# muhtutorials/wireguard

Hardware: AMD Instinct MI355X
Metric: device-resident payload GiB/s, Internet checksum, 64k×1500B batch (higher is better)
Workload: dtype u8; 1 GPU; 65536 x 1500-B tcp4 frames per GPU, validate (checksumValid, gro.go:554-612) per step, BASELINE.json configs[1]; packets_per_gpu=65536, frame_len=1500, global_batch_bytes=98304000, mode=validate, rotated_copies=4, frame_stride=1500, streams=2, parallelism=shard1 (no collective)

## Files before the change

wireguard_amd/csrc/api.cpp:

```cpp
#include <hip/hip_runtime.h>

#include <algorithm>

#include <cstdarg>
#include <cstdio>
#include <cstdlib>
#include <cstring>
#include <mutex>
#include <string>

#include "../../include/wgcsum.h"
#include "wgcs_ctx.h"
#include "wgcs_kernels.h"

using namespace wgcs;

namespace wgcs {

namespace {
thread_local const wgcs_ctx* tls_err_ctx = nullptr;
thread_local char tls_err[512];
}

int set_err(wgcs_ctx* ctx, int code, const char* fmt, ...) {
  if (ctx) {
    va_list ap;
    va_start(ap, fmt);
    vsnprintf(tls_err, sizeof tls_err, fmt, ap);
    va_end(ap);
    tls_err_ctx = ctx;
  }
  return code;
}

int hip_fail(wgcs_ctx* ctx, hipError_t e, const char* what) {
  return set_err(ctx, WGCS_ERR_HIP, "%s: %s", what, hipGetErrorString(e));
}

int ensure_dev(wgcs_ctx* ctx, DevBuf& b, size_t bytes) {
  if (bytes <= b.cap) return WGCS_OK;
  if (b.ptr) hipFree(b.ptr);
  b.ptr = nullptr;
  b.cap = 0;
  size_t want = bytes < 4096 ? 4096 : bytes + bytes / 4;
  hipError_t e = hipMalloc(&b.ptr, want);
  if (e != hipSuccess) return hip_fail(ctx, e, "hipMalloc");
  b.cap = want;
  return WGCS_OK;
}

int ensure_pinned(wgcs_ctx* ctx, HostBuf& b, size_t bytes) {
  if (bytes <= b.cap) return WGCS_OK;
  if (b.ptr) hipHostFree(b.ptr);
  b.ptr = nullptr;
  b.cap = 0;
  size_t want = bytes < 4096 ? 4096 : bytes + bytes / 4;
  hipError_t e = hipHostMalloc(&b.ptr, want, hipHostMallocDefault);
  if (e != hipSuccess) return hip_fail(ctx, e, "hipHostMalloc");
  void* d = nullptr;
  e = hipHostGetDevicePointer(&d, b.ptr, 0);
  if (e != hipSuccess || d != b.ptr) {
    hipHostFree(b.ptr);
    b.ptr = nullptr;
    return e != hipSuccess ? hip_fail(ctx, e, "hipHostGetDevicePointer")
                           : set_err(ctx, WGCS_ERR_HIP, "pinned memory is not mapped at its host address");
  }
  b.cap = want;
  return WGCS_OK;
}

bool host_mapped_locked(wgcs_ctx* ctx, const void* p, size_t n) {
  const uintptr_t a = (uintptr_t)p, b = a + n;
  for (const auto& r : ctx->host_allocs)
    if (a >= r.first && b <= r.second && b >= a) return true;
  return false;
}

bool host_mapped(wgcs_ctx* ctx, const void* p, size_t n) {
  std::lock_guard<std::mutex> g(ctx->host_mu);
  return host_mapped_locked(ctx, p, n);
}

}

extern "C" {

int wgcs_abi_version(void) { return WGCS_ABI_VERSION; }

int wgcs_device_count(int* count) {
  if (!count) return WGCS_ERR_INVALID_ARG;
  int n = 0;
  hipError_t e = hipGetDeviceCount(&n);
  if (e != hipSuccess) {
    *count = 0;
    return WGCS_ERR_NO_DEVICE;
  }
  *count = n;
  return WGCS_OK;
}

int wgcs_init(int device, wgcs_ctx** out) {
  if (!out) return WGCS_ERR_INVALID_ARG;
  *out = nullptr;
  int n = 0;
  if (hipGetDeviceCount(&n) != hipSuccess || n <= 0) return WGCS_ERR_NO_DEVICE;
  if (device < 0 || device >= n) return WGCS_ERR_INVALID_ARG;
  wgcs_ctx* ctx = new (std::nothrow) wgcs_ctx();
  if (!ctx) return WGCS_ERR_NOMEM;
  ctx->device = device;
  hipError_t e = hipSetDevice(device);
  if (e == hipSuccess) e = hipStreamCreateWithFlags(&ctx->stream, hipStreamDefault);
  hipDeviceProp_t prop;
  if (e == hipSuccess) e = hipGetDeviceProperties(&prop, device);
  for (int j = 1; j < WGCS_MAX_BATCH_STREAMS && e == hipSuccess; ++j)
    e = hipEventCreateWithFlags(&ctx->join_ev[j], hipEventDisableTiming);
  if (e != hipSuccess) {
    for (hipEvent_t ev : ctx->join_ev)
      if (ev) hipEventDestroy(ev);
    if (ctx->stream) hipStreamDestroy(ctx->stream);
    delete ctx;
    return WGCS_ERR_HIP;
  }
  ctx->num_cu = prop.multiProcessorCount;
  const char* bpc = getenv("WGCS_BLOCKS_PER_CU");
  if (bpc && atoi(bpc) > 0) ctx->tune.blocks_per_cu = atoi(bpc);
  const char* unr = getenv("WGCS_UNROLL");
  if (unr && atoi(unr) > 0) ctx->tune.unroll = atoi(unr);
  const char* lpp = getenv("WGCS_LANES_PER_PKT");
  if (lpp && (atoi(lpp) == 64 || atoi(lpp) == 32 || atoi(lpp) == 16)) ctx->tune.lanes_per_pkt = atoi(lpp);
  const char* nt = getenv("WGCS_NT");
  if (nt) ctx->tune.nt = atoi(nt) ? 1 : 0;
  const char* xc = getenv("WGCS_XCD");
  if (xc) ctx->tune.xcd = atoi(xc) ? 1 : 0;
  const char* al = getenv("WGCS_ALIGN");
  if (al && (atoi(al) == 16 || atoi(al) == 32 || atoi(al) == 64 || atoi(al) == 128)) ctx->tune.align = atoi(al);
  *out = ctx;
  return WGCS_OK;
}

int wgcs_host_alloc(wgcs_ctx* ctx, size_t bytes, void** p) {
  if (!ctx || !p || bytes == 0) return WGCS_ERR_INVALID_ARG;
  *p = nullptr;
  hipSetDevice(ctx->device);
  const size_t n = (bytes + 15) & ~(size_t)15;
  void* h = nullptr;
  hipError_t e = hipHostMalloc(&h, n, hipHostMallocCoherent);
  if (e != hipSuccess) return hip_fail(ctx, e, "wgcs_host_alloc");
  void* d = nullptr;
  e = hipHostGetDevicePointer(&d, h, 0);
  if (e != hipSuccess || d != h) {
    hipHostFree(h);
    return e != hipSuccess ? hip_fail(ctx, e, "hipHostGetDevicePointer")
                           : set_err(ctx, WGCS_ERR_HIP, "pinned memory is not mapped at its host address");
  }
  std::lock_guard<std::mutex> g(ctx->host_mu);
  ctx->host_allocs.emplace_back((uintptr_t)h, (uintptr_t)h + n);
  *p = h;
  return WGCS_OK;
}

int wgcs_host_free(wgcs_ctx* ctx, void* p) {
  if (!ctx || !p) return WGCS_ERR_INVALID_ARG;
  {
    std::lock_guard<std::mutex> g(ctx->host_mu);
    auto& v = ctx->host_allocs;
    auto it = std::find_if(v.begin(), v.end(), [&](const std::pair<uintptr_t, uintptr_t>& r) {
      return r.first == (uintptr_t)p;
    });
    if (it == v.end()) return set_err(ctx, WGCS_ERR_INVALID_ARG, "wgcs_host_free: not a wgcs_host_alloc pointer");
    for (wgcs_wstager* ws : ctx->wstagers)
      if (wstager_references(ws, it->first, it->second))
        return set_err(ctx, WGCS_ERR_NOT_READY, "wgcs_host_free: a write-stager slot still reads this memory");
    v.erase(it);
  }
  const hipError_t e = hipHostFree(p);
  return e == hipSuccess ? WGCS_OK : hip_fail(ctx, e, "hipHostFree");
}

int wgcs_destroy(wgcs_ctx* ctx) {
  if (!ctx) return WGCS_ERR_INVALID_ARG;
  {
    std::lock_guard<std::mutex> g(ctx->host_mu);
    if (!ctx->wstagers.empty() || !ctx->stagers.empty())
      return set_err(ctx, WGCS_ERR_INVALID_ARG,
                     "wgcs_destroy: %zu read stager(s) and %zu write stager(s) still alive: destroy them first",
                     ctx->stagers.size(), ctx->wstagers.size());
  }
  hipSetDevice(ctx->device);
  if (ctx->stream) hipStreamSynchronize(ctx->stream);
  for (const auto& r : ctx->host_allocs) hipHostFree((void*)r.first);
  for (DevBuf* b : {&ctx->d_arena, &ctx->d_pkts, &ctx->d_init, &ctx->d_out, &ctx->d_out2, &ctx->d_aux})
    if (b->ptr) hipFree(b->ptr);
  for (HostBuf* b : {&ctx->h_stage, &ctx->h_meta, &ctx->h_out})
    if (b->ptr) hipHostFree(b->ptr);
  if (ctx->stream) hipStreamDestroy(ctx->stream);
  for (hipEvent_t ev : ctx->join_ev)
    if (ev) hipEventDestroy(ev);
  delete ctx;
  return WGCS_OK;
}

const char* wgcs_strerror(int status) {
  switch (status) {
    case WGCS_OK: return "ok";
    case WGCS_ERR_INVALID_ARG: return "invalid argument";
    case WGCS_ERR_SHORT_BUFFER: return "short buffer";
    case WGCS_ERR_TOO_MANY_SEGMENTS: return "too many segments";
    case WGCS_ERR_INVALID_OFFSET: return "invalid offset";
    case WGCS_ERR_UNSUPPORTED_GSO: return "unsupported virtio GSO type";
    case WGCS_ERR_IP_GSO_MISMATCH: return "IP header version / GSO type mismatch";
    case WGCS_ERR_BAD_IP_VERSION: return "invalid IP header version";
    case WGCS_ERR_PACKET_TOO_SHORT: return "packet is too short";
    case WGCS_ERR_TCP_HDR_LEN: return "TCP header length is invalid";
    case WGCS_ERR_HDR_LEN: return "length of packet < virtioNetHdr.hdrLen";
    case WGCS_ERR_CSUM_OFFSET: return "end of checksum offset exceeds packet length";
    case WGCS_ERR_READ_OVERFLOW: return "read length overflows bufs element length";
    case WGCS_ERR_OUT_OF_RANGE: return "slice bounds out of range";
    case WGCS_ERR_BATCH_FULL: return "staging batch full";
    case WGCS_ERR_NOT_READY: return "batch not submitted or already recycled";
    case WGCS_ERR_CMSG: return "error parsing socket control message";
    case WGCS_ERR_SPLIT_OVERFLOW: return "splitting coalesced packet resulted in overflow";
    case WGCS_ERR_AUTH: return "chacha20poly1305: message authentication failed";
    case WGCS_ERR_SOURCE: return "packet with disallowed source address";
    case WGCS_ERR_REPLAY: return "replayed or out-of-window counter";
    case WGCS_ERR_MAC1: return "received packet with invalid mac1";
    case WGCS_ERR_LOW_ORDER: return "bad input point: low order point";
    case WGCS_ERR_NO_PEER: return "no running peer with this public key";
    case WGCS_ERR_HIP: return "HIP runtime error";
    case WGCS_ERR_NOMEM: return "out of memory";
    case WGCS_ERR_NO_DEVICE: return "no HIP device";
    default: return "unknown status";
  }
}

const char* wgcs_last_error(wgcs_ctx* ctx) { return ctx && tls_err_ctx == ctx ? tls_err : ""; }

int wgcs_num_cu(wgcs_ctx* ctx) { return ctx ? ctx->num_cu : WGCS_ERR_INVALID_ARG; }

int wgcs_sync(wgcs_ctx* ctx) {
  if (!ctx) return WGCS_ERR_INVALID_ARG;
  std::lock_guard<std::mutex> g(ctx->mu);
  hipSetDevice(ctx->device);
  hipError_t e = hipStreamSynchronize(ctx->stream);
  return e == hipSuccess ? WGCS_OK : hip_fail(ctx, e, "hipStreamSynchronize");
}

int wgcs_checksum_batch(wgcs_ctx* ctx, int mode, unsigned flags, uint8_t* d_arena, const wgcs_pkt* d_pkts,
                        const uint64_t* d_initial, uint32_t n, void* d_out, void* stream) {
  if (!ctx) return WGCS_ERR_INVALID_ARG;
  if (mode < WGCS_MODE_FOLD || mode > WGCS_MODE_IP4HDR) return set_err(ctx, WGCS_ERR_INVALID_ARG, "bad mode %d", mode);
  if (n == 0) return WGCS_OK;
  if (!d_arena || !d_pkts || !d_out) return set_err(ctx, WGCS_ERR_INVALID_ARG, "NULL pointer");
  std::lock_guard<std::mutex> g(ctx->mu);
  hipSetDevice(ctx->device);
  hipStream_t s = stream ? (hipStream_t)stream : ctx->stream;
  hipError_t e = launch_checksum_batch(mode, flags, d_arena, d_pkts, d_initial, n, d_out, s, ctx->num_cu, ctx->tune);
  return e == hipSuccess ? WGCS_OK : hip_fail(ctx, e, "checksum_batch launch");
}

int wgcs_checksum_batches(wgcs_ctx* ctx, int mode, unsigned flags, const wgcs_batch* batches, uint32_t n_batches,
                          void* const* streams, uint32_t n_streams, void* ev_begin, void* ev_end) {
  if (!ctx) return WGCS_ERR_INVALID_ARG;
  if (mode < WGCS_MODE_FOLD || mode > WGCS_MODE_IP4HDR) return set_err(ctx, WGCS_ERR_INVALID_ARG, "bad mode %d", mode);
  if (n_streams > WGCS_MAX_BATCH_STREAMS || (n_streams && !streams) || (n_batches && !batches))
    return set_err(ctx, WGCS_ERR_INVALID_ARG, "bad stream list (%u streams)", n_streams);
  for (uint32_t k = 0; k < n_batches; ++k)
    if (batches[k].n && (!batches[k].arena || !batches[k].pkts || !batches[k].out))
      return set_err(ctx, WGCS_ERR_INVALID_ARG, "batch %u: NULL pointer", k);
  std::lock_guard<std::mutex> g(ctx->mu);
  hipSetDevice(ctx->device);
  const uint32_t ns = n_streams ? n_streams : 1;
  hipStream_t st[WGCS_MAX_BATCH_STREAMS];
  for (uint32_t j = 0; j < ns; ++j) st[j] = n_streams && streams[j] ? (hipStream_t)streams[j] : ctx->stream;
  hipError_t e = hipSuccess;
  if (ev_begin && (e = hipEventRecord((hipEvent_t)ev_begin, st[0])) != hipSuccess) return hip_fail(ctx, e, "ev_begin");
  for (uint32_t k = 0; k < n_batches; ++k) {
    const uint32_t j = k % ns;
    if (ev_begin && j != 0 && k < ns && st[j] != st[0] &&
        (e = hipStreamWaitEvent(st[j], (hipEvent_t)ev_begin, 0)) != hipSuccess)
      return hip_fail(ctx, e, "stream wait");
    const wgcs_batch& b = batches[k];
    e = launch_checksum_batch(mode, flags, b.arena, b.pkts, b.initial, b.n, b.out, st[j], ctx->num_cu, ctx->tune);
    if (e != hipSuccess) return hip_fail(ctx, e, "checksum_batches launch");
  }
  if (ev_end) {
    const uint32_t used = n_batches < ns ? n_batches : ns;
    for (uint32_t j = 1; j < used; ++j) {
      if (st[j] == st[0]) continue;
      if ((e = hipEventRecord(ctx->join_ev[j], st[j])) != hipSuccess ||
          (e = hipStreamWaitEvent(st[0], ctx->join_ev[j], 0)) != hipSuccess)
        return hip_fail(ctx, e, "stream join");
    }
    if ((e = hipEventRecord((hipEvent_t)ev_end, st[0])) != hipSuccess) return hip_fail(ctx, e, "ev_end");
  }
  return WGCS_OK;
}

int wgcs_stream_wait_flag(wgcs_ctx* ctx, void* stream, const uint32_t* flag, uint32_t value) {
  if (!ctx || !flag || ((uintptr_t)flag & 3u)) return WGCS_ERR_INVALID_ARG;
  if (!host_mapped(ctx, flag, sizeof(uint32_t)))
    return set_err(ctx, WGCS_ERR_INVALID_ARG, "wgcs_stream_wait_flag: flag is not wgcs_host_alloc memory");
  std::lock_guard<std::mutex> g(ctx->mu);
  hipSetDevice(ctx->device);
  hipStream_t s = stream ? (hipStream_t)stream : ctx->stream;
  const hipError_t e = hipStreamWaitValue32(s, const_cast<uint32_t*>(flag), value, hipStreamWaitValueEq, 0xFFFFFFFFu);
  return e == hipSuccess ? WGCS_OK : hip_fail(ctx, e, "hipStreamWaitValue32");
}

constexpr size_t kZeroCopyMax = 1u << 20;

int wgcs_checksum_batch_host(wgcs_ctx* ctx, int mode, unsigned flags, uint8_t* h_arena, size_t arena_len,
                             const wgcs_pkt* h_pkts, const uint64_t* h_initial, uint32_t n, void* h_out) {
  if (!ctx) return WGCS_ERR_INVALID_ARG;
  if (mode < WGCS_MODE_FOLD || mode > WGCS_MODE_IP4HDR) return set_err(ctx, WGCS_ERR_INVALID_ARG, "bad mode %d", mode);
  if (n == 0) return WGCS_OK;
  if (!h_pkts || !h_out || (!h_arena && arena_len)) return set_err(ctx, WGCS_ERR_INVALID_ARG, "NULL pointer");
  for (uint32_t i = 0; i < n; ++i) {
    const uint64_t off = (uint64_t)h_pkts[i].off_lo | ((uint64_t)h_pkts[i].off_hi << 32);
    if (h_pkts[i].len >= 0x80000000u || off + h_pkts[i].len > arena_len)
      return set_err(ctx, WGCS_ERR_INVALID_ARG, "packet %u outside the arena", i);
    const size_t addr_end = (h_pkts[i].flags & WGCS_PKT_V6) ? 40 : 20;
    if ((mode == WGCS_MODE_VALIDATE || mode == WGCS_MODE_L4_FILL) && off + addr_end > arena_len)
      return set_err(ctx, WGCS_ERR_OUT_OF_RANGE, "packet %u: pseudo-header addresses past the arena", i);
  }
  std::lock_guard<std::mutex> g(ctx->mu);
  hipSetDevice(ctx->device);
  const size_t out_bytes = (size_t)n * (mode == WGCS_MODE_VALIDATE ? 1 : 2);
  int rc;
  const bool fold_init = h_initial && mode == WGCS_MODE_FOLD;
  if (arena_len <= kZeroCopyMax) {
    auto al = [](size_t x) { return (x + 15) & ~(size_t)15; };
    const size_t o_pk = al(arena_len) + 16, o_in = o_pk + al(n * sizeof(wgcs_pkt)),
                 o_out = o_in + (fold_init ? al(n * sizeof(uint64_t)) : 0);
    if ((rc = ensure_pinned(ctx, ctx->h_stage, o_out + al(out_bytes) + 16))) return rc;
    uint8_t* hs = (uint8_t*)ctx->h_stage.ptr;
    if (arena_len) memcpy(hs, h_arena, arena_len);
    memcpy(hs + o_pk, h_pkts, n * sizeof(wgcs_pkt));
    if (fold_init) memcpy(hs + o_in, h_initial, n * sizeof(uint64_t));
    hipError_t e = launch_checksum_batch(mode, flags, hs, (const wgcs_pkt*)(hs + o_pk),
                                         fold_init ? (const uint64_t*)(hs + o_in) : nullptr, n, hs + o_out,
                                         ctx->stream, ctx->num_cu, ctx->tune);
    if (e != hipSuccess) return hip_fail(ctx, e, "checksum_batch launch");
    if ((e = hipStreamSynchronize(ctx->stream)) != hipSuccess) return hip_fail(ctx, e, "checksum_batch wait");
    memcpy(h_out, hs + o_out, out_bytes);
    if ((flags & WGCS_F_INPLACE) && arena_len) memcpy(h_arena, hs, arena_len);
    return WGCS_OK;
  }
  if ((rc = ensure_dev(ctx, ctx->d_arena, arena_len + 16)) || (rc = ensure_dev(ctx, ctx->d_pkts, n * sizeof(wgcs_pkt))) ||
      (rc = ensure_dev(ctx, ctx->d_out, out_bytes)))
    return rc;
  if (fold_init && (rc = ensure_dev(ctx, ctx->d_init, n * sizeof(uint64_t)))) return rc;
  hipStream_t s = ctx->stream;
  hipError_t e = hipMemcpyAsync(ctx->d_arena.ptr, h_arena, arena_len, hipMemcpyHostToDevice, s);
  if (e == hipSuccess) e = hipMemcpyAsync(ctx->d_pkts.ptr, h_pkts, n * sizeof(wgcs_pkt), hipMemcpyHostToDevice, s);
  const uint64_t* dinit = nullptr;
  if (e == hipSuccess && h_initial && mode == WGCS_MODE_FOLD) {
    e = hipMemcpyAsync(ctx->d_init.ptr, h_initial, n * sizeof(uint64_t), hipMemcpyHostToDevice, s);
    dinit = (const uint64_t*)ctx->d_init.ptr;
  }
  if (e != hipSuccess) return hip_fail(ctx, e, "H2D");
  e = launch_checksum_batch(mode, flags, (uint8_t*)ctx->d_arena.ptr, (const wgcs_pkt*)ctx->d_pkts.ptr, dinit, n,
                            ctx->d_out.ptr, s, ctx->num_cu, ctx->tune);
  if (e != hipSuccess) return hip_fail(ctx, e, "checksum_batch launch");
  e = hipMemcpyAsync(h_out, ctx->d_out.ptr, out_bytes, hipMemcpyDeviceToHost, s);
  if (e == hipSuccess && (flags & WGCS_F_INPLACE) && arena_len)
    e = hipMemcpyAsync(h_arena, ctx->d_arena.ptr, arena_len, hipMemcpyDeviceToHost, s);
  if (e == hipSuccess) e = hipStreamSynchronize(s);
  return e == hipSuccess ? WGCS_OK : hip_fail(ctx, e, "D2H");
}

int wgcs_checksum(wgcs_ctx* ctx, const uint8_t* b, size_t n, uint64_t initial, uint16_t* out) {
  if (!ctx || !out || (!b && n)) return WGCS_ERR_INVALID_ARG;
  if (n >= 0x80000000u) return set_err(ctx, WGCS_ERR_INVALID_ARG, "buffer too large");
  wgcs_pkt p;
  wgcs_pkt_set(&p, 0, (uint32_t)n, 0, 0, 0, 0);
  return wgcs_checksum_batch_host(ctx, WGCS_MODE_FOLD, 0, const_cast<uint8_t*>(b), n, &p, &initial, 1, out);
}

int wgcs_checksum_valid_cap(wgcs_ctx* ctx, const uint8_t* pkt, size_t len, size_t cap, uint8_t iph_len, uint8_t proto,
                            int is_v6, int* valid) {
  if (!ctx || !valid || (!pkt && cap) || cap < len) return WGCS_ERR_INVALID_ARG;
  const size_t need = is_v6 ? 40 : 20;
  if (cap < need || len < iph_len)
    return set_err(ctx, WGCS_ERR_OUT_OF_RANGE, "pkt[%u:] or its addresses past the slice", (unsigned)iph_len);
  if (len >= 0x80000000u) return set_err(ctx, WGCS_ERR_INVALID_ARG, "packet too large");
  wgcs_pkt p;
  wgcs_pkt_set(&p, 0, (uint32_t)len, iph_len, 0, proto, (uint8_t)(is_v6 ? WGCS_PKT_V6 : 0));
  uint8_t v = 0;
  int rc = wgcs_checksum_batch_host(ctx, WGCS_MODE_VALIDATE, 0, const_cast<uint8_t*>(pkt), std::max(len, need), &p,
                                    nullptr, 1, &v);
  *valid = v;
  return rc;
}

int wgcs_checksum_valid(wgcs_ctx* ctx, const uint8_t* pkt, size_t len, uint8_t iph_len, uint8_t proto, int is_v6,
                        int* valid) {
  return wgcs_checksum_valid_cap(ctx, pkt, len, len, iph_len, proto, is_v6, valid);
}

int wgcs_gso_none_checksum(wgcs_ctx* ctx, uint8_t* read_buf, size_t len, uint16_t csum_start, uint16_t csum_offset) {
  if (!ctx || (!read_buf && len)) return WGCS_ERR_INVALID_ARG;
  const uint16_t at = (uint16_t)(csum_start + csum_offset);
  if ((size_t)at + 2 > len || csum_start > len)
    return set_err(ctx, WGCS_ERR_OUT_OF_RANGE, "checksum field %u outside packet of %zu bytes", at, len);
  if (len >= 0x80000000u) return set_err(ctx, WGCS_ERR_INVALID_ARG, "packet too large");
  wgcs_pkt p;
  wgcs_pkt_set(&p, 0, (uint32_t)len, csum_start, csum_offset, 0, 0);
  uint16_t out = 0;
  return wgcs_checksum_batch_host(ctx, WGCS_MODE_PARTIAL, WGCS_F_INPLACE, read_buf, len, &p, nullptr, 1, &out);
}

}
```

wireguard_amd/csrc/checksum_kernels.hip:

```cpp
#include <hip/hip_runtime.h>

#include "../../include/wgcsum.h"
#include "wgcs_common.h"
#include "wgcs_kernels.h"

namespace wgcs {

struct Ranges {
  int main_lo, main_hi;
  int addr_lo, addr_hi;
  int fld;
};

__device__ __forceinline__ uint32_t edge_chunk(uint32_t acc, const uint4& v, int pos, const Ranges& r, bool rot_addr,
                                               bool addr) {
  const int f = r.fld - pos;
  uint32_t fb = 0;
  if (f >= -1 && f < 16) fb = ((3u << (f + 1)) >> 1) & 0xFFFFu;
  const uint32_t m16 = byte_bits16(r.main_lo - pos, r.main_hi - pos) & ~fb;
  const uint32_t w[4] = {v.x, v.y, v.z, v.w};
#pragma unroll
  for (int k = 0; k < 4; ++k) acc = add_halves(acc, w[k] & expand_nibble((m16 >> (4 * k)) & 0xFu));
  if (addr) {
    const uint32_t a16 = byte_bits16(r.addr_lo - pos, r.addr_hi - pos) & ~fb;
#pragma unroll
    for (int k = 0; k < 4; ++k) {
      uint32_t y = w[k] & expand_nibble((a16 >> (4 * k)) & 0xFu);
      if (rot_addr) y = rotl8(y);
      acc = add_halves(acc, y);
    }
  }
  return acc;
}

template <bool NT>
__device__ __forceinline__ uint4 ld_chunk(const uint4* p) {
  if (NT) {
    typedef unsigned int u32x4 __attribute__((ext_vector_type(4)));
    const u32x4 t = __builtin_nontemporal_load(reinterpret_cast<const u32x4*>(p));
    return make_uint4(t.x, t.y, t.z, t.w);
  }
  return *p;
}

struct Desc {
  uint64_t off;
  int len, cs, co, proto, flags;
};
__device__ __forceinline__ Desc unpack(const uint4& d) {
  Desc r;
  r.off = (uint64_t)d.x | ((uint64_t)(d.y & 0xFFFFu) << 32);
  r.proto = (int)((d.y >> 16) & 0xFFu);
  r.flags = (int)(d.y >> 24);
  r.len = (int)d.z;
  r.cs = (int)(d.w & 0xFFFFu);
  r.co = (int)(d.w >> 16);
  return r;
}

template <int PPW>
__device__ __forceinline__ uint4 wave_desc(const uint4* __restrict__ pkts, uint32_t base, uint32_t n, int grp) {
  uint4 d[PPW];
#pragma unroll
  for (int k = 0; k < PPW; ++k) d[k] = (base + (uint32_t)k < n) ? pkts[base + k] : make_uint4(0, 0, 0, 0);
  uint4 r = d[0];
#pragma unroll
  for (int k = 1; k < PPW; ++k)
    if (grp == k) r = d[k];
  return r;
}

#ifndef WGCS_CS_ACC2
#define WGCS_CS_ACC2 1
#endif
#ifndef WGCS_CS_MERGE
#define WGCS_CS_MERGE 1
#endif
#ifndef WGCS_CS_BLOCK
#define WGCS_CS_BLOCK 256
#endif
template <int MODE, int G, int U, bool NT>
__global__ __launch_bounds__(WGCS_CS_BLOCK) void checksum_batch_kernel(uint8_t* __restrict__ arena,
                                                             const uint4* __restrict__ pkts,
                                                             const uint64_t* __restrict__ initial,
                                                             uint32_t n, void* __restrict__ out,
                                                             int inplace, uint32_t amask, int xcd) {
  static_assert(G == 16 || G == 32 || G == 64, "group = DPP row, half wave or wave");
  constexpr int PPW = 64 / G;
  const int lane = threadIdx.x & 63;
  const int grp = lane / G;
  const int sub = lane % G;
  uint32_t blk = blockIdx.x;
  if (xcd) blk = (blk & 7u) * (gridDim.x >> 3) + (blk >> 3);
  const uint32_t wave = (uint32_t)__builtin_amdgcn_readfirstlane((int)(blk * (blockDim.x >> 6) + (threadIdx.x >> 6)));
  const uint32_t step = gridDim.x * (blockDim.x >> 6) * PPW;
  uint4 dn = wave_desc<PPW>(pkts, wave * PPW, n, grp);
  for (uint32_t base = wave * PPW; base < n; base += step) {
    const uint32_t p = base + grp;
    const bool active = p < n;
    const Desc d = unpack(dn);
    if (p + step < n) dn = pkts[p + step];
    uint8_t* pkt = arena + d.off;
    const int len = active ? d.len : 0;
    const int cs = d.cs;
    const bool v6 = (d.flags & WGCS_PKT_V6) != 0;
    const int fld16 = (cs + d.co) & 0xFFFF;
    Ranges r;
    r.main_lo = 0;
    r.main_hi = len;
    r.addr_lo = 0;
    r.addr_hi = 0;
    r.fld = -1000000;
    uint32_t pre = 0;
    uint64_t init = 0;
    if (MODE == WGCS_MODE_FOLD) {
      init = (initial && active) ? initial[p] : 0;
    } else if (MODE == WGCS_MODE_L4_FILL || MODE == WGCS_MODE_VALIDATE) {
      r.main_lo = min(cs, len);
      r.addr_lo = v6 ? 8 : 12;
      r.addr_hi = v6 ? 40 : 20;
      if (MODE == WGCS_MODE_L4_FILL) r.fld = fld16;
      pre = (uint32_t)d.proto + ((uint32_t)(len - cs) & 0xFFFFu);
    } else if (MODE == WGCS_MODE_PARTIAL) {
      r.main_lo = min(cs, len);
      r.fld = fld16;
      if (r.fld + 1 < len) init = ((uint32_t)pkt[r.fld] << 8) | pkt[r.fld + 1];
    } else {
      r.main_hi = min(cs, len);
      r.fld = 10;
    }
#if WGCS_CS_MERGE
    if (r.addr_hi > r.addr_lo && r.addr_hi == r.main_lo && ((r.addr_lo ^ r.main_lo) & 1) == 0) {
      r.main_lo = r.addr_lo;
      r.addr_lo = r.addr_hi = 0;
    }
#endif
    const bool any_addr = __builtin_amdgcn_ballot_w64(r.addr_hi > r.addr_lo) != 0;
    const uintptr_t pbase = (uintptr_t)pkt;
    const bool rot_addr = (((pbase + r.addr_lo) ^ (pbase + r.main_lo)) & 1u) != 0;
    int lo_all = r.main_lo, hi_all = r.main_hi, hole_end = r.main_lo;
    if (r.addr_hi > r.addr_lo) {
      lo_all = min(lo_all, r.addr_lo);
      hi_all = max(hi_all, r.addr_hi);
      hole_end = max(hole_end, r.addr_hi);
    }
    if (r.fld + 2 > lo_all && r.fld < hi_all) hole_end = max(hole_end, r.fld + 2);
    const int rel0 = lo_all - (int)((pbase + (uintptr_t)lo_all) & amask);
    const int nch = hi_all > lo_all ? (hi_all - rel0 + 15) >> 4 : 0;
    int c_lo = min((hole_end - rel0 + 15) >> 4, nch);
    int c_hi = nch ? max((hi_all - rel0) >> 4, c_lo) : 0;
    const int n_edge = c_lo + (nch - c_hi);
    const uint4* __restrict__ src = reinterpret_cast<const uint4*>(pkt + rel0);
    uint32_t acc = 0;
    int ce = sub < c_lo ? sub : c_hi + (sub - c_lo);
    uint4 ve = (sub < n_edge && rel0 + 16 * ce + 16 > lo_all) ? ld_chunk<NT>(src + ce) : make_uint4(0, 0, 0, 0);
    bool edge_pending = true;
    const int c_it = amask >= 127u ? (c_lo & ~7) : c_lo;
    for (int c0 = c_it + sub; c0 < c_hi || edge_pending; c0 += G * U) {
      uint4 v[U];
#pragma unroll
      for (int u = 0; u < U; ++u) {
        const int c = c0 + u * G;
        v[u] = (c < c_hi && c >= c_lo) ? ld_chunk<NT>(src + c) : make_uint4(0, 0, 0, 0);
      }
      if (edge_pending) {
        for (int e = sub;;) {
          if (e < n_edge) acc = edge_chunk(acc, ve, rel0 + 16 * ce, r, rot_addr, any_addr);
          e += G;
          if (e >= n_edge) break;
          ce = e < c_lo ? e : c_hi + (e - c_lo);
          ve = rel0 + 16 * ce + 16 > lo_all ? ld_chunk<NT>(src + ce) : make_uint4(0, 0, 0, 0);
        }
        edge_pending = false;
      }
      acc = (acc >> 16) + (acc & 0xFFFFu);
#if WGCS_CS_ACC2
      uint32_t acc2 = 0;
#pragma unroll
      for (int u = 0; u < U; ++u) {
        acc = add_halves(acc, v[u].x);
        acc2 = add_halves(acc2, v[u].z);
        acc = add_halves(acc, v[u].y);
        acc2 = add_halves(acc2, v[u].w);
      }
      acc += acc2;
#else
#pragma unroll
      for (int u = 0; u < U; ++u) {
        acc = add_halves(acc, v[u].x);
        acc = add_halves(acc, v[u].y);
        acc = add_halves(acc, v[u].z);
        acc = add_halves(acc, v[u].w);
      }
#endif
    }
    uint32_t s = fold32_16(acc);
    if (G == 16) {
      s = row16_sum_u32(s);
    } else if (G == 32) {
      s = row16_sum_u32(s);
      s += (uint32_t)__shfl_xor((int)s, 16);
    } else {
      s = wave_sum_u32(s);
    }
    s = fold32_16(s);
    if (((pbase + (uintptr_t)r.main_lo) & 1u) == 0) s = bswap16(s);
    uint32_t t = fold32_16(s + pre + fold64_16(init));
    const bool past = (MODE == WGCS_MODE_L4_FILL || MODE == WGCS_MODE_VALIDATE) && cs > len;
    if (sub == 0 && active) {
      if (MODE == WGCS_MODE_VALIDATE) {
        reinterpret_cast<uint8_t*>(out)[p] = (t == 0xFFFFu && !past) ? 1 : 0;
      } else if (MODE == WGCS_MODE_FOLD) {
        reinterpret_cast<uint16_t*>(out)[p] = (uint16_t)t;
      } else {
        const uint16_t c = past ? (uint16_t)0 : (uint16_t)~t;
        reinterpret_cast<uint16_t*>(out)[p] = c;
        if (inplace && !past && r.fld >= 0 && r.fld + 1 < len) {
          pkt[r.fld] = (uint8_t)(c >> 8);
          pkt[r.fld + 1] = (uint8_t)c;
        }
      }
    }
  }
}

template <int MODE>
static hipError_t launch_mode(uint8_t* arena, const wgcs_pkt* pkts, const uint64_t* init, uint32_t n, void* out,
                              int inplace, hipStream_t s, int num_cu, const LaunchTuning& t) {
  const int ppb = (64 / t.lanes_per_pkt) * (WGCS_CS_BLOCK / 64);
  long want = ((long)n + ppb - 1) / ppb;
  want = (want + 7) & ~7L;
  long cap = (long)num_cu * t.blocks_per_cu;
  cap = cap > 8 ? cap & ~7L : cap;
  const int grid = (int)(want < cap ? want : cap);
  const uint32_t amask = (uint32_t)(t.align >= 16 ? t.align : 16) - 1u;
  const int xcd = (t.xcd && grid % 8 == 0) ? 1 : 0;
  const uint4* d = reinterpret_cast<const uint4*>(pkts);
#define WGCS_LAUNCH(G, U)                                                                                    \
  do {                                                                                                      \
    if (t.nt)                                                                                               \
      hipLaunchKernelGGL((checksum_batch_kernel<MODE, G, U, true>), dim3(grid), dim3(WGCS_CS_BLOCK), 0, s, arena, d, \
                         init, n, out, inplace, amask, xcd);                                                \
    else                                                                                                    \
      hipLaunchKernelGGL((checksum_batch_kernel<MODE, G, U, false>), dim3(grid), dim3(WGCS_CS_BLOCK), 0, s, arena, d, \
                         init, n, out, inplace, amask, xcd);                                                \
  } while (0)
  if (t.lanes_per_pkt == 64) {
    if (t.unroll >= 4) WGCS_LAUNCH(64, 4);
    else WGCS_LAUNCH(64, 2);
  } else if (t.lanes_per_pkt == 32) {
    if (t.unroll >= 6) WGCS_LAUNCH(32, 6);
    else if (t.unroll >= 4) WGCS_LAUNCH(32, 4);
    else WGCS_LAUNCH(32, 3);
  } else {
    if (t.unroll >= 8) WGCS_LAUNCH(16, 8);
    else if (t.unroll >= 6) WGCS_LAUNCH(16, 6);
    else WGCS_LAUNCH(16, 4);
  }
#undef WGCS_LAUNCH
  return hipGetLastError();
}

hipError_t launch_checksum_batch(int mode, unsigned flags, uint8_t* arena, const wgcs_pkt* pkts,
                                 const uint64_t* init, uint32_t n, void* out, hipStream_t s, int num_cu,
                                 const LaunchTuning& tune) {
  if (n == 0) return hipSuccess;
  const int inplace = (flags & WGCS_F_INPLACE) ? 1 : 0;
  switch (mode) {
    case WGCS_MODE_FOLD:
      return launch_mode<WGCS_MODE_FOLD>(arena, pkts, init, n, out, inplace, s, num_cu, tune);
    case WGCS_MODE_L4_FILL:
      return launch_mode<WGCS_MODE_L4_FILL>(arena, pkts, init, n, out, inplace, s, num_cu, tune);
    case WGCS_MODE_VALIDATE:
      return launch_mode<WGCS_MODE_VALIDATE>(arena, pkts, init, n, out, inplace, s, num_cu, tune);
    case WGCS_MODE_PARTIAL:
      return launch_mode<WGCS_MODE_PARTIAL>(arena, pkts, init, n, out, inplace, s, num_cu, tune);
    case WGCS_MODE_IP4HDR:
      return launch_mode<WGCS_MODE_IP4HDR>(arena, pkts, init, n, out, inplace, s, num_cu, tune);
    default:
      return hipErrorInvalidValue;
  }
}

}
```

wireguard_amd/csrc/wgcs_ctx.h:

```cpp
#pragma once

#include <hip/hip_runtime.h>

#include <mutex>
#include <string>
#include <utility>
#include <vector>

#include "../../include/wgcsum.h"
#include "wgcs_kernels.h"

namespace wgcs {

struct DevBuf {
  void* ptr = nullptr;
  size_t cap = 0;
};
struct HostBuf {
  void* ptr = nullptr;
  size_t cap = 0;
};

int set_err(wgcs_ctx* ctx, int code, const char* fmt, ...);
int hip_fail(wgcs_ctx* ctx, hipError_t e, const char* what);
int ensure_dev(wgcs_ctx* ctx, DevBuf& b, size_t bytes);
int ensure_pinned(wgcs_ctx* ctx, HostBuf& b, size_t bytes);
bool host_mapped(wgcs_ctx* ctx, const void* p, size_t n);
bool host_mapped_locked(wgcs_ctx* ctx, const void* p, size_t n);
bool wstager_references(wgcs_wstager* ws, uintptr_t a, uintptr_t b);
int gso_split_staged(wgcs_ctx* ctx, const uint8_t* vbuf, size_t vlen, uint32_t jflags, uint8_t* const* bufs,
                     const size_t* buf_lens, int nbufs, int* sizes, int offset, int* status, int* count);

int ring_gso_prepare(wgcs_ring* rg, uint32_t kbufs, size_t region, uint8_t** hs, int32_t** meta);
int ring_gso(wgcs_ring* rg, const uint8_t* vbuf, uint32_t vlen, uint32_t jflags, uint32_t kbufs, uint32_t pitch,
             uint32_t room, uint32_t posflags, uint8_t* out, int32_t* meta);
bool ring_mapped(wgcs_ring* rg, const void* p, size_t n);
int ring_input(wgcs_ring* rg, const uint8_t* p, size_t n, const uint8_t** out);
std::mutex& ring_mutex(wgcs_ring* rg);
wgcs_ctx* ring_ctx(wgcs_ring* rg);

}

struct wgcs_ctx {
  int device = 0;
  int num_cu = 256;
  hipStream_t stream = nullptr;
  std::mutex mu;
  wgcs::LaunchTuning tune;
  wgcs::DevBuf d_arena, d_pkts, d_init, d_out, d_out2, d_aux;
  wgcs::HostBuf h_stage, h_meta, h_out;
  hipEvent_t join_ev[WGCS_MAX_BATCH_STREAMS] = {};
  std::mutex host_mu;
  std::vector<std::pair<uintptr_t, uintptr_t>> host_allocs;
  std::vector<wgcs_wstager*> wstagers;
  std::vector<wgcs_stager*> stagers;
};
```

wireguard_amd/csrc/wgcs_kernels.h:

```cpp
#pragma once

#include <hip/hip_runtime.h>
#include <stdint.h>

#include "../../include/wgcsum.h"
#include "wgcs_host.h"

namespace wgcs {

hipError_t launch_checksum_batch(int mode, unsigned flags, uint8_t* arena, const wgcs_pkt* pkts,
                                 const uint64_t* init, uint32_t n, void* out, hipStream_t s, int num_cu,
                                 const LaunchTuning& tune);

hipError_t launch_ring(RingCtl* ctl, uint32_t nb, uint32_t last, uint64_t idle_ticks, hipStream_t s);
void gso_kernel_shape(int* lds_waves, int* parts, int* u, int* rows);
hipError_t launch_gso_split_batch(const uint8_t* arena, const wgcs_gso_job* jobs, uint32_t n_jobs,
                                  uint8_t* out, uint32_t out_stride, uint32_t offset, uint32_t max_segs,
                                  int32_t* sizes, int32_t* count, int32_t* status,
                                  hipStream_t s, const GsoOutPos* outpos = nullptr, uint32_t room = 0);

hipError_t launch_gro_batch(uint8_t* arena, wgcs_gro_buf* bufs, const wgcs_gro_call* calls, uint32_t n_calls,
                            int32_t* status, int32_t* n_write, int32_t* to_write, hipStream_t s);

hipError_t launch_ws_scatter(const uint8_t* stage, uint8_t* arena, const WsMove* mv, uint32_t n, hipStream_t s);
hipError_t launch_ws_gather(const uint8_t* arena, const wgcs_gro_buf* bufs, const wgcs_gro_call* calls,
                            const WsOut* outs, uint32_t n_calls, int32_t* status, const int32_t* n_write,
                            const int32_t* to_write, int32_t* wlen, int32_t* wpos, uint8_t* out, hipStream_t s);

hipError_t launch_gro_coalesce(const uint8_t* stage, const GroItem* items, uint32_t n_items, const GroSeg* segs,
                               uint32_t n_segs, uint8_t* out, hipStream_t s);

hipError_t launch_udp_split(const uint8_t* in, uint64_t in_stride, uint32_t buf_len, const int32_t* n_in,
                            const int32_t* gso, uint32_t n_msgs, uint32_t first, uint32_t n_batches, uint8_t* out,
                            uint64_t out_stride, int32_t* n_out, int32_t* src, int32_t* count, int32_t* status,
                            hipStream_t s);
hipError_t launch_udp_coalesce(uint8_t* bufs, uint64_t stride, uint32_t buf_cap, const int32_t* caps,
                               const int32_t* lens, const int32_t* nbufs, uint32_t max_bufs, uint32_t n_batches,
                               int dst_is_v6, int32_t* n_msgs, int32_t* msg_first, int32_t* msg_len,
                               int32_t* msg_gso, hipStream_t s);

hipError_t launch_aead_batch(int open, uint8_t* arena, const wgcs_aead_pkt* pkts, const wgcs_aead_key* keys,
                             uint32_t n_keys, uint32_t n, uint32_t mtu, int32_t* out_len, uint64_t* out_ctr,
                             hipStream_t s);

hipError_t launch_recv_classify(const uint8_t* arena, const uint64_t* off, uint64_t stride, const int32_t* sizes,
                                uint32_t n, const wgcs_session_slot* slots, uint32_t n_slots, wgcs_aead_pkt* pkts,
                                int32_t* types, hipStream_t s);
hipError_t launch_recv_source(const uint8_t* arena, const wgcs_aead_pkt* pkts, const int32_t* pkt_len,
                              const uint32_t* key_peer, uint32_t n_keys, uint32_t n, const uint8_t* image,
                              uint64_t image_bytes, int32_t* verdict, uint32_t* peer, hipStream_t s);
hipError_t launch_route_dst(const uint8_t* arena, const uint64_t* off, uint64_t stride, uint32_t offset,
                            const int32_t* sizes, uint32_t n, const uint8_t* image, uint64_t image_bytes,
                            uint32_t* peer, hipStream_t s);

struct KeyOrder;
hipError_t launch_replay(const KeyOrder& ko, const wgcs_aead_pkt* pkts, const int32_t* pkt_len,
                         const uint64_t* counter, uint32_t n, wgcs_replay_filter* filters, uint32_t n_keys,
                         uint64_t limit, int32_t* verdict, hipStream_t s);
hipError_t launch_send_assign(const KeyOrder& ko, const int32_t* sizes, const uint32_t* peer, const int32_t* count,
                              const int32_t* status, uint32_t n_jobs, uint32_t max_segs, uint64_t stride,
                              const wgcs_session_slot* peer_keys, uint32_t n_slots, uint64_t* send_nonce,
                              uint32_t n_keys, uint64_t limit, wgcs_aead_pkt* pkts, int32_t* nbufs, uint32_t* job_key,
                              hipStream_t s);

hipError_t launch_write_build(const wgcs_aead_pkt* pkts, const int32_t* verdict, uint32_t n_msgs, uint32_t n_batches,
                              const uint32_t* key_peer, uint32_t n_keys, int32_t offset, uint32_t cap,
                              uint32_t gro_flags, uint32_t calls_per_batch, wgcs_gro_buf* bufs, wgcs_gro_call* calls,
                              wgcs_write_group* groups, int32_t* n_groups, int32_t* status, hipStream_t s);

hipError_t launch_hs_screen(const uint8_t* arena, const wgcs_aead_pkt* pkts, const int32_t* types, uint32_t n,
                            const wgcs_cookie_checker* checker, const wgcs_src_addr* srcs, uint32_t under_load,
                            const uint8_t* nonces, int32_t* verdict, uint8_t* replies, hipStream_t s);

hipError_t launch_x25519(const uint8_t* scalars, const uint8_t* points, uint32_t n, uint8_t* out, int32_t* status,
                         hipStream_t s);
hipError_t launch_hs_consume(const uint8_t* arena, const wgcs_aead_pkt* pkts, const int32_t* types,
                             const int32_t* gate, uint32_t n, const wgcs_noise_responder* responder,
                             const wgcs_peer_key* table, uint32_t n_peers, int32_t* verdict, wgcs_hs_init* out,
                             hipStream_t s);

}
```

Measured before the change: 6041 GiB/s.

## Fuse multiple checksum batches into one grouped kernel launch on a single stream

Measured after the change: 6481 GiB/s, median of 6. 1.07x the previous value.

```diff
diff --git a/wireguard_amd/csrc/api.cpp b/wireguard_amd/csrc/api.cpp
--- a/wireguard_amd/csrc/api.cpp
+++ b/wireguard_amd/csrc/api.cpp
@@ -114,9 +114,11 @@
   if (e == hipSuccess) e = hipGetDeviceProperties(&prop, device);
   for (int j = 1; j < WGCS_MAX_BATCH_STREAMS && e == hipSuccess; ++j)
     e = hipEventCreateWithFlags(&ctx->join_ev[j], hipEventDisableTiming);
+  if (e == hipSuccess) e = hipEventCreateWithFlags(&ctx->fork_ev, hipEventDisableTiming);
   if (e != hipSuccess) {
     for (hipEvent_t ev : ctx->join_ev)
       if (ev) hipEventDestroy(ev);
+    if (ctx->fork_ev) hipEventDestroy(ctx->fork_ev);
     if (ctx->stream) hipStreamDestroy(ctx->stream);
     delete ctx;
     return WGCS_ERR_HIP;
@@ -134,6 +136,7 @@
   if (xc) ctx->tune.xcd = atoi(xc) ? 1 : 0;
   const char* al = getenv("WGCS_ALIGN");
   if (al && (atoi(al) == 16 || atoi(al) == 32 || atoi(al) == 64 || atoi(al) == 128)) ctx->tune.align = atoi(al);
+  ctx->fuse = batch_plan_fuse_env(getenv("WGCS_FUSE"));
   *out = ctx;
   return WGCS_OK;
 }
@@ -196,6 +199,7 @@
   if (ctx->stream) hipStreamDestroy(ctx->stream);
   for (hipEvent_t ev : ctx->join_ev)
     if (ev) hipEventDestroy(ev);
+  if (ctx->fork_ev) hipEventDestroy(ctx->fork_ev);
   delete ctx;
   return WGCS_OK;
 }
@@ -274,6 +278,38 @@
   for (uint32_t j = 0; j < ns; ++j) st[j] = n_streams && streams[j] ? (hipStream_t)streams[j] : ctx->stream;
   hipError_t e = hipSuccess;
   if (ev_begin && (e = hipEventRecord((hipEvent_t)ev_begin, st[0])) != hipSuccess) return hip_fail(ctx, e, "ev_begin");
+  const BatchPlanCfg cfg = {(uint32_t)checksum_pkts_per_block(ctx->tune), (uint64_t)ctx->num_cu * ctx->tune.blocks_per_cu,
+                            ctx->fuse};
+  if (batch_plan_fusable(flags, cfg)) {
+    const uint32_t used = n_batches < ns ? n_batches : ns;
+    for (uint32_t j = 1; j < used; ++j) {
+      if (st[j] == st[0]) continue;
+      if ((e = hipEventRecord(ctx->join_ev[j], st[j])) != hipSuccess ||
+          (e = hipStreamWaitEvent(st[0], ctx->join_ev[j], 0)) != hipSuccess)
+        return hip_fail(ctx, e, "stream join");
+    }
+    BatchTable tab;
+    uint32_t idx[kBatchGroupMax];
+    for (uint32_t k = 0; k < n_batches;) {
+      k = batch_plan_next(batches, n_batches, k, mode, cfg, &tab, idx);
+      if (tab.count == 1) {
+        const BatchEntry& b = tab.e[0];
+        e = launch_checksum_batch(mode, flags, b.arena, b.pkts, b.initial, b.n, b.out, st[0], ctx->num_cu, ctx->tune);
+      } else {
+        e = launch_checksum_group(mode, tab, st[0], ctx->tune);
+      }
+      if (e != hipSuccess) return hip_fail(ctx, e, "checksum_batches launch");
+    }
+    bool forked = false;
+    for (uint32_t j = 1; j < used; ++j) {
+      if (st[j] == st[0]) continue;
+      if (!forked && (e = hipEventRecord(ctx->fork_ev, st[0])) != hipSuccess) return hip_fail(ctx, e, "stream fork");
+      forked = true;
+      if ((e = hipStreamWaitEvent(st[j], ctx->fork_ev, 0)) != hipSuccess) return hip_fail(ctx, e, "stream fork");
+    }
+    if (ev_end && (e = hipEventRecord((hipEvent_t)ev_end, st[0])) != hipSuccess) return hip_fail(ctx, e, "ev_end");
+    return WGCS_OK;
+  }
   for (uint32_t k = 0; k < n_batches; ++k) {
     const uint32_t j = k % ns;
     if (ev_begin && j != 0 && k < ns && st[j] != st[0] &&
diff --git a/wireguard_amd/csrc/checksum_kernels.hip b/wireguard_amd/csrc/checksum_kernels.hip
--- a/wireguard_amd/csrc/checksum_kernels.hip
+++ b/wireguard_amd/csrc/checksum_kernels.hip
@@ -1,6 +1,7 @@
 #include <hip/hip_runtime.h>
 
 #include "../../include/wgcsum.h"
+#include "wgcs_batch_plan.h"
 #include "wgcs_common.h"
 #include "wgcs_kernels.h"
 
@@ -80,20 +81,18 @@
 #define WGCS_CS_BLOCK 256
 #endif
 template <int MODE, int G, int U, bool NT>
-__global__ __launch_bounds__(WGCS_CS_BLOCK) void checksum_batch_kernel(uint8_t* __restrict__ arena,
-                                                             const uint4* __restrict__ pkts,
-                                                             const uint64_t* __restrict__ initial,
-                                                             uint32_t n, void* __restrict__ out,
-                                                             int inplace, uint32_t amask, int xcd) {
+__device__ __forceinline__ void checksum_batch_body(uint8_t* __restrict__ arena, const uint4* __restrict__ pkts,
+                                                    const uint64_t* __restrict__ initial, uint32_t n,
+                                                    void* __restrict__ out, int inplace, uint32_t amask, int xcd,
+                                                    uint32_t blk, const uint32_t nblk) {
   static_assert(G == 16 || G == 32 || G == 64, "group = DPP row, half wave or wave");
   constexpr int PPW = 64 / G;
   const int lane = threadIdx.x & 63;
   const int grp = lane / G;
   const int sub = lane % G;
-  uint32_t blk = blockIdx.x;
-  if (xcd) blk = (blk & 7u) * (gridDim.x >> 3) + (blk >> 3);
+  if (xcd) blk = (blk & 7u) * (nblk >> 3) + (blk >> 3);
   const uint32_t wave = (uint32_t)__builtin_amdgcn_readfirstlane((int)(blk * (blockDim.x >> 6) + (threadIdx.x >> 6)));
-  const uint32_t step = gridDim.x * (blockDim.x >> 6) * PPW;
+  const uint32_t step = nblk * (blockDim.x >> 6) * PPW;
   uint4 dn = wave_desc<PPW>(pkts, wave * PPW, n, grp);
   for (uint32_t base = wave * PPW; base < n; base += step) {
     const uint32_t p = base + grp;
@@ -224,6 +223,31 @@
   }
 }
 
+template <int MODE, int G, int U, bool NT>
+__global__ __launch_bounds__(WGCS_CS_BLOCK) void checksum_batch_kernel(uint8_t* __restrict__ arena,
+                                                             const uint4* __restrict__ pkts,
+                                                             const uint64_t* __restrict__ initial,
+                                                             uint32_t n, void* __restrict__ out,
+                                                             int inplace, uint32_t amask, int xcd) {
+  checksum_batch_body<MODE, G, U, NT>(arena, pkts, initial, n, out, inplace, amask, xcd, blockIdx.x, gridDim.x);
+}
+
+template <int MODE, int G, int U, bool NT>
+__global__ __launch_bounds__(WGCS_CS_BLOCK) void checksum_batch_kernel(const BatchTable t, uint32_t amask, int xcd) {
+  const uint32_t bi = blockIdx.x;
+  uint32_t e;
+  if (t.same_shift != kBatchNoEntry) {
+    e = bi >> t.same_shift;
+  } else {
+    e = 0;
+#pragma unroll
+    for (uint32_t k = 1; k < kBatchGroupMax; ++k) e = bi >= t.first[k] ? k : e;
+  }
+  const BatchEntry& b = t.e[e];
+  checksum_batch_body<MODE, G, U, NT>(b.arena, reinterpret_cast<const uint4*>(b.pkts), b.initial, b.n, b.out, 0, amask,
+                                      xcd, bi - b.first, b.blocks);
+}
+
 template <int MODE>
 static hipError_t launch_mode(uint8_t* arena, const wgcs_pkt* pkts, const uint64_t* init, uint32_t n, void* out,
                               int inplace, hipStream_t s, int num_cu, const LaunchTuning& t) {
@@ -261,6 +285,55 @@
   return hipGetLastError();
 }
 
+template <int MODE>
+static hipError_t launch_group_mode(const BatchTable& tab, hipStream_t s, const LaunchTuning& t) {
+  const uint32_t amask = (uint32_t)(t.align >= 16 ? t.align : 16) - 1u;
+  const int xcd = t.xcd ? 1 : 0;
+#define WGCS_LAUNCH(G, U)                                                                                          \
+  do {                                                                                                            \
+    if (t.nt)                                                                                                     \
+      hipLaunchKernelGGL((checksum_batch_kernel<MODE, G, U, true>), dim3(tab.total), dim3(WGCS_CS_BLOCK), 0, s, tab, \
+                         amask, xcd);                                                                             \
+    else                                                                                                          \
+      hipLaunchKernelGGL((checksum_batch_kernel<MODE, G, U, false>), dim3(tab.total), dim3(WGCS_CS_BLOCK), 0, s, tab, \
+                         amask, xcd);                                                                             \
+  } while (0)
+  if (t.lanes_per_pkt == 64) {
+    if (t.unroll >= 4) WGCS_LAUNCH(64, 4);
+    else WGCS_LAUNCH(64, 2);
+  } else if (t.lanes_per_pkt == 32) {
+    if (t.unroll >= 6) WGCS_LAUNCH(32, 6);
+    else if (t.unroll >= 4) WGCS_LAUNCH(32, 4);
+    else WGCS_LAUNCH(32, 3);
+  } else {
+    if (t.unroll >= 8) WGCS_LAUNCH(16, 8);
+    else if (t.unroll >= 6) WGCS_LAUNCH(16, 6);
+    else WGCS_LAUNCH(16, 4);
+  }
+#undef WGCS_LAUNCH
+  return hipGetLastError();
+}
+
+int checksum_pkts_per_block(const LaunchTuning& t) { return (64 / t.lanes_per_pkt) * (WGCS_CS_BLOCK / 64); }
+
+hipError_t launch_checksum_group(int mode, const BatchTable& tab, hipStream_t s, const LaunchTuning& tune) {
+  if (tab.count == 0 || tab.total == 0) return hipSuccess;
+  switch (mode) {
+    case WGCS_MODE_FOLD:
+      return launch_group_mode<WGCS_MODE_FOLD>(tab, s, tune);
+    case WGCS_MODE_L4_FILL:
+      return launch_group_mode<WGCS_MODE_L4_FILL>(tab, s, tune);
+    case WGCS_MODE_VALIDATE:
+      return launch_group_mode<WGCS_MODE_VALIDATE>(tab, s, tune);
+    case WGCS_MODE_PARTIAL:
+      return launch_group_mode<WGCS_MODE_PARTIAL>(tab, s, tune);
+    case WGCS_MODE_IP4HDR:
+      return launch_group_mode<WGCS_MODE_IP4HDR>(tab, s, tune);
+    default:
+      return hipErrorInvalidValue;
+  }
+}
+
 hipError_t launch_checksum_batch(int mode, unsigned flags, uint8_t* arena, const wgcs_pkt* pkts,
                                  const uint64_t* init, uint32_t n, void* out, hipStream_t s, int num_cu,
                                  const LaunchTuning& tune) {
diff --git a/wireguard_amd/csrc/wgcs_batch_plan.h b/wireguard_amd/csrc/wgcs_batch_plan.h
--- /dev/null
+++ b/wireguard_amd/csrc/wgcs_batch_plan.h
@@ -0,0 +1,119 @@
+#pragma once
+
+#include <stddef.h>
+#include <stdint.h>
+
+#include "../../include/wgcsum.h"
+
+namespace wgcs {
+
+constexpr uint32_t kBatchGroupMax = 32;
+constexpr uint32_t kBatchNoEntry = 0xFFFFFFFFu;
+
+struct BatchEntry {
+  uint8_t* arena;
+  const wgcs_pkt* pkts;
+  const uint64_t* initial;
+  void* out;
+  uint32_t n;
+  uint32_t blocks;
+  uint32_t first;
+  uint32_t pad;
+};
+struct BatchTable {
+  uint32_t first[kBatchGroupMax];
+  BatchEntry e[kBatchGroupMax];
+  uint32_t count;
+  uint32_t total;
+  uint32_t same_shift;
+  uint32_t pad;
+};
+static_assert(sizeof(BatchEntry) == 48 && sizeof(BatchTable) == 128 + 32 * 48 + 16, "table layout");
+
+struct BatchPlanCfg {
+  uint32_t pkts_per_block;
+  uint64_t cap;
+  bool fuse;
+};
+
+inline bool batch_plan_fuse_env(const char* v) {
+  if (!v) return true;
+  while (*v == ' ') ++v;
+  return !(v[0] == '0' && v[1] == '\0');
+}
+
+inline uint32_t batch_out_width(int mode) { return mode == WGCS_MODE_VALIDATE ? 1u : 2u; }
+
+inline uint32_t batch_plan_cap8(const BatchPlanCfg& c) {
+  const uint64_t lim = (uint64_t)0x7FFFFFF8u / kBatchGroupMax;
+  const uint64_t cap = c.cap < lim ? c.cap : lim;
+  return (uint32_t)(cap & ~(uint64_t)7);
+}
+
+inline bool batch_plan_fusable(unsigned flags, const BatchPlanCfg& c) {
+  return c.fuse && !(flags & WGCS_F_INPLACE) && c.pkts_per_block > 0 && batch_plan_cap8(c) >= 8;
+}
+
+inline uint32_t batch_plan_blocks(uint32_t n, const BatchPlanCfg& c) {
+  uint64_t want = ((uint64_t)n + c.pkts_per_block - 1) / c.pkts_per_block;
+  want = (want + 7) & ~(uint64_t)7;
+  const uint32_t cap = batch_plan_cap8(c);
+  return want < cap ? (uint32_t)want : cap;
+}
+
+inline bool batch_same_tuple(const wgcs_batch& a, const wgcs_batch& b) {
+  return a.arena == b.arena && a.pkts == b.pkts && a.initial == b.initial && a.out == b.out && a.n == b.n;
+}
+
+inline bool batch_may_share(const wgcs_batch& a, const wgcs_batch& b, uint32_t w) {
+  const uintptr_t a0 = (uintptr_t)a.out, a1 = a0 + (uintptr_t)a.n * w;
+  const uintptr_t b0 = (uintptr_t)b.out, b1 = b0 + (uintptr_t)b.n * w;
+  return a1 <= b0 || b1 <= a0 || batch_same_tuple(a, b);
+}
+
+inline uint32_t batch_plan_next(const wgcs_batch* batches, uint32_t n_batches, uint32_t k0, int mode,
+                                const BatchPlanCfg& c, BatchTable* tab, uint32_t* idx) {
+  const uint32_t w = batch_out_width(mode);
+  uint32_t cnt = 0, total = 0, k = k0;
+  for (; k < n_batches && cnt < kBatchGroupMax; ++k) {
+    const wgcs_batch& b = batches[k];
+    if (b.n == 0) continue;
+    bool ok = true;
+    for (uint32_t e = 0; e < cnt && ok; ++e) ok = batch_may_share(batches[idx[e]], b, w);
+    if (!ok) break;
+    BatchEntry& t = tab->e[cnt];
+    t.arena = b.arena;
+    t.pkts = b.pkts;
+    t.initial = b.initial;
+    t.out = b.out;
+    t.n = b.n;
+    t.blocks = batch_plan_blocks(b.n, c);
+    t.first = total;
+    t.pad = 0;
+    tab->first[cnt] = total;
+    idx[cnt] = k;
+    total += t.blocks;
+    ++cnt;
+  }
+  for (uint32_t e = cnt; e < kBatchGroupMax; ++e) {
+    tab->first[e] = kBatchNoEntry;
+    tab->e[e] = BatchEntry{nullptr, nullptr, nullptr, nullptr, 0, 0, kBatchNoEntry, 0};
+  }
+  tab->count = cnt;
+  tab->total = total;
+  tab->same_shift = kBatchNoEntry;
+  if (cnt) {
+    const uint32_t nb = tab->e[0].blocks;
+    bool same = (nb & (nb - 1)) == 0;
+    for (uint32_t e = 1; e < cnt && same; ++e) same = tab->e[e].blocks == nb;
+    if (same) {
+      uint32_t s = 0;
+      while ((1u << s) < nb) ++s;
+      tab->same_shift = s;
+    }
+  }
+  tab->pad = 0;
+  return k;
+}
+
+}
diff --git a/wireguard_amd/csrc/wgcs_ctx.h b/wireguard_amd/csrc/wgcs_ctx.h
--- a/wireguard_amd/csrc/wgcs_ctx.h
+++ b/wireguard_amd/csrc/wgcs_ctx.h
@@ -50,6 +50,8 @@
   wgcs::DevBuf d_arena, d_pkts, d_init, d_out, d_out2, d_aux;
   wgcs::HostBuf h_stage, h_meta, h_out;
   hipEvent_t join_ev[WGCS_MAX_BATCH_STREAMS] = {};
+  hipEvent_t fork_ev = nullptr;
+  bool fuse = true;
   std::mutex host_mu;
   std::vector<std::pair<uintptr_t, uintptr_t>> host_allocs;
   std::vector<wgcs_wstager*> wstagers;
diff --git a/wireguard_amd/csrc/wgcs_kernels.h b/wireguard_amd/csrc/wgcs_kernels.h
--- a/wireguard_amd/csrc/wgcs_kernels.h
+++ b/wireguard_amd/csrc/wgcs_kernels.h
@@ -4,6 +4,7 @@
 #include <stdint.h>
 
 #include "../../include/wgcsum.h"
+#include "wgcs_batch_plan.h"
 #include "wgcs_host.h"
 
 namespace wgcs {
@@ -11,6 +12,8 @@
 hipError_t launch_checksum_batch(int mode, unsigned flags, uint8_t* arena, const wgcs_pkt* pkts,
                                  const uint64_t* init, uint32_t n, void* out, hipStream_t s, int num_cu,
                                  const LaunchTuning& tune);
+hipError_t launch_checksum_group(int mode, const BatchTable& tab, hipStream_t s, const LaunchTuning& tune);
+int checksum_pkts_per_block(const LaunchTuning& tune);
 
 hipError_t launch_ring(RingCtl* ctl, uint32_t nb, uint32_t last, uint64_t idle_ticks, hipStream_t s);
 void gso_kernel_shape(int* lds_waves, int* parts, int* u, int* rows);
```
